# ThomasK33/kube-scheduler-simulator

Hardware: AMD Instinct MI355X
Metric: pod x node filter+score evals/sec (higher is better)
Workload: dtype int64

## Files before the change

### kube-scheduler-simulator_amd/csrc/ksim_batch.hip

```cpp
#include "ksim_device.h"
#include <atomic>

#include "ksim_internal.h"
#include "ksim_wave.h"
#include "ksim_commit.h"
#include "ksim_chain.h"

namespace ksim {



template <int kTopThreads, int N = kTileCand, bool SORTED = true>
__device__ __forceinline__ void top_finish(uint64_t (&a)[N], int32_t nfeas, int32_t j,
                                           uint64_t* __restrict__ topk, int32_t* __restrict__ topk_cnt,
                                           int32_t* __restrict__ topk_complete, uint64_t* __restrict__ xsend,
                                           uint64_t* tclk = nullptr) {
  constexpr int kTopWaves = kTopThreads / 64;
  constexpr int kTopSlots = (kTopWaves * kTopT + 63) / 64;
  __shared__ uint64_t s_list[kTopWaves][kTopT];
  __shared__ int32_t s_cnt[kTopWaves], s_complete[kTopWaves];
  const int lane = threadIdx.x & 63, wv = threadIdx.x >> 6;
  {
    __shared__ uint64_t s_wmax[kTopWaves], s_wthr[kTopWaves];
    __shared__ int32_t s_wf[kTopWaves], s_ncand;
// ... 713 lines not shown
                                          int32_t end) {
  PodRec r{};
  if (q < end) {
    const ksim_pod& y = P.pods[q];
    r.req = PodReq{y.req_cpu, y.req_mem, y.req_eph, y.nz_cpu, y.nz_mem};
    r.cls = rcls[q];
    r.valid = 1;
  }
  return r;
}

template <bool FLUSH, bool DIRECT, bool DEF, bool KEEP, bool NS, bool RT = false>
__device__ __forceinline__ void batch_top_commit_body(const DevCluster& c, const DevPods& P,
                                                      const ksim_profile* __restrict__ prof_p,
                                                      const BatchProg* __restrict__ bp_p, const LazyStep& L,
                                                      uint64_t* __restrict__ topk, int32_t* __restrict__ topk_cnt,
                                                      int32_t* __restrict__ topk_complete,
                                                      int32_t* __restrict__ chosen_out,
                                                      uint64_t* __restrict__ xsend, const ReqTab& rt = ReqTab{}) {
  constexpr int kThreads = 1024;
  static_assert(kThreads >= kBatchPods, "one thread per batch entry");
  static_assert(!RT || (DIRECT && !NS && (FLUSH || (DEF && KEEP))), "the table form is the KEEP / DEF / DIRECT launch");
  static_assert(2 * kReqMaxClasses <= kThreads, "upkeep: one thread per (class, row)");
  __shared__ uint16_t s_cls[RT ? kBatchPods + 1 : 1];
  __shared__ uint16_t s_patch[RT ? kBatchPods + 1 : 1];
  __shared__ UpRow s_up[RT ? 2 : 1];
  __shared__ ResCols s_rq[kBatchPods + 1];
  __shared__ PodReq s_pc[kBatchPods + (NS ? kNsPods : 1)];
  __shared__ __attribute__((aligned(16))) int16_t s_ent[DIRECT ? kLazyDirect : 1];
  __shared__ int32_t s_hkey[DIRECT ? 1 : kLazyHash];
  __shared__ int16_t s_hval[DIRECT ? 1 : kLazyHash];
  __shared__ uint32_t s_bits[DIRECT ? 1 : kLazyBitWords];
  __shared__ int32_t s_istar, s_inode, s_sched, s_unsched;
  const int tid = threadIdx.x;
  const int32_t b = blockIdx.x;
  const int32_t pod0 = NS ? (b / kNsSlices) * kNsPods : b;
#ifdef KSIM_TC_CLOCKS
  const uint64_t t_in = __builtin_amdgcn_s_memrealtime();
  uint64_t t_pro = 0, t_loop = 0, tclk[4] = {0, 0, 0, 0}, tp[3] = {0, 0, 0};
#endif
  const int32_t e1 = *L.e1, e2 = *L.e2;
  uint64_t g1 = 0, m1 = 0, g2 = 0;
  if (tid < kBatchPods) {
    g1 = L.g1[tid];
    m1 = L.m1[tid];
  }
  if (tid == b) g2 = L.g2[b];
  const int32_t cur0 = L.st_in->cursor, end = L.st_in->end;
  const int64_t seq0 = L.st_in->pod_seq;
  ResCols rq{0, 0, 0, 0, 0, 0};
  if constexpr (RT) {
    static_assert(2 * kBatchPods + 1 <= kThreads, "one record per thread");
    if (tid < 2 * kBatchPods + 1) {
      const PodRec r = load_rec(rt.h_in + (tid < kBatchPods ? tid : b + (tid - kBatchPods)));
      if (tid < kBatchPods) {
        rq = ResCols{r.req.cpu, r.req.mem, r.req.eph, r.req.nzc, r.req.nzm, (int32_t)r.valid};
      } else {
        s_pc[tid - kBatchPods] = r.req;
        s_cls[tid - kBatchPods] = r.valid ? r.cls : kNoClass;
      }
    }
  } else {
    for (int x = tid; x < 2 * kBatchPods + (NS ? kNsPods : 1); x += kThreads) {
      const int32_t q = x < kBatchPods ? cur0 + x : cur0 + pod0 + (x - kBatchPods);
      if (q < end) {
        const ksim_pod& y = P.pods[q];
// ... 6 lines not shown
    }
  }
  if constexpr (DIRECT) {
    const uint64_t fill = 0x0001000100010001ull * (uint64_t)kBatchPods;
    for (int x = tid; x < (c.n + 3) >> 2; x += kThreads) reinterpret_cast<uint64_t*>(s_ent)[x] = fill;
  } else {
    const int nwords = (c.n + 31) >> 5;
    for (int x = tid; x < kLazyHash; x += kThreads) s_hkey[x] = -1;
    for (int x = tid; x < nwords; x += kThreads) s_bits[x] = 0;
  }
  const int32_t nchain = e1 > 0 ? e1 : 0;
  if (tid == 0) {
    s_istar = nchain;
    s_inode = -1;
    s_sched = 0;
    s_unsched = 0;
    s_rq[kBatchPods] = ResCols{0, 0, 0, 0, 0, 0};
  }
  PodReq creq{0, 0, 0, 0, 0};
  if constexpr (RT) {
    const int32_t t = tid < 64 ? 0 : tid - 64;
    creq = rt.rreq[t < 2 * rt.n_cls ? (t < rt.n_cls ? t : t - rt.n_cls) : 0];
  }
  lds_barrier();
#ifdef KSIM_TC_CLOCKS
  tp[0] = __builtin_amdgcn_s_memrealtime();
#endif
  block_first_min(&s_istar, tid < nchain && m1 > g1);
  lds_barrier();
#ifdef KSIM_TC_CLOCKS
  tp[1] = __builtin_amdgcn_s_memrealtime();
#endif
  const int32_t istar = s_istar;
  const int32_t committed = istar < nchain ? istar + 1 : nchain;
  if (tid == istar && istar < nchain) s_inode = key_node(m1) - c.base;
  if (tid < committed) s_rq[tid] = rq;
  const int32_t base = cur0 + committed;
  const int32_t pi = base + pod0;
  const bool live = !FLUSH && pi < min(end, base + kBatchPods);
  const int rl = tid - (kThreads - 128);
  const bool rec_writer = RT && rl >= 0 && rl < (int)(sizeof(PodRec) / 8);
  lds_barrier();
#ifdef KSIM_TC_CLOCKS
  tp[2] = __builtin_amdgcn_s_memrealtime();
#endif
  const int32_t inode = s_inode;
  const int32_t gnode = (tid < istar && g1) ? key_node(g1) - c.base : -1;
  uint32_t te[kKeepPerLane];
  uint32_t pe = 0;
  NodeRow prow{};
  double pic = 0, pim = 0;
  const bool twice = RT && !FLUSH && live && gnode >= 0 && gnode == inode;
  if constexpr (RT && !FLUSH) {
    const int32_t cls = live ? (int32_t)s_cls[committed] : 0;
    if (live && gnode >= 0) pe = rt.p_in[(size_t)cls * kBatchPods + tid];
    if (twice) {
      prow = load_res_row_off(c, gnode);
      pic = ld_off(c.inv_cpu, (uint32_t)gnode << 3);
      pim = ld_off(c.inv_mem, (uint32_t)gnode << 3);
    }
    const uint16_t* __restrict__ trow = rt.t_in + (size_t)cls * (size_t)c.n;
#pragma unroll
    for (int q = 0; q < kKeepPerLane; q++) {
      const int32_t node = c.eval_lo + tid + q * kThreads;
      te[q] = trow[node < c.eval_hi ? node : c.eval_lo];
    }
  }
  if (gnode >= 0) {
    ResCols d = rq;
    if (gnode == inode) {
      const ResCols x = s_rq[istar];
      d.cpu += x.cpu;
      d.mem += x.mem;
      d.eph += x.eph;
      d.nzc += x.nzc;
      d.nzm += x.nzm;
      d.pods += 1;
    }
    s_rq[tid] = d;
    if constexpr (RT && !FLUSH) {
// ... 36 lines not shown
    if (mn0 >= 0) mr0 = ResCols{c.req_cpu[mn0], c.req_mem[mn0], c.req_eph[mn0], c.nz_cpu[mn0], c.nz_mem[mn0], c.num_pods[mn0]};
    if (mn1 >= 0) mr1 = ResCols{c.req_cpu[mn1], c.req_mem[mn1], c.req_eph[mn1], c.nz_cpu[mn1], c.nz_mem[mn1], c.num_pods[mn1]};
    if constexpr (RT) {
      const int32_t mn[2] = {mn0, mn1};
#pragma unroll
      for (int w = 0; w < 2; w++) {
        const int32_t n = mn[w] >= 0 ? mn[w] : 0;
        ms[w].alloc_cpu = c.alloc_cpu[n];
        ms[w].alloc_mem = c.alloc_mem[n];
        ms[w].alloc_eph = c.alloc_eph[n];
        ms[w].inv_cpu = c.inv_cpu[n];
        ms[w].inv_mem = c.inv_mem[n];
        ms[w].alloc_pods = c.alloc_pods[n];
        ms[w].node = mn[w];
      }
    }
  }
  lds_barrier();
  auto update_state = [&]() {
    static_assert(sizeof(DevState) % 8 == 0, "DevState by words");
    constexpr int kWords = (int)(sizeof(DevState) / 8);
    uint64_t w[kWords];
#pragma unroll
    for (int q = 0; q < kWords; q++) w[q] = reinterpret_cast<const uint64_t*>(L.st_in)[q];
    DevState ns;
    __builtin_memcpy(&ns, w, sizeof(ns));
    if (e1 > 0) {
      const int32_t nb = min(kBatchPods, end - cur0);
      ns.cursor = base;
      ns.pod_seq = seq0 + committed;
      ns.scheduled += s_sched;
      ns.unschedulable += s_unsched;
      ns.batches += 1;
      ns.cuts += (committed < nb && istar < nchain ? 1 : 0);
      ns.truncations += (committed < nb && istar >= nchain ? 1 : 0);
      ns.evals += (int64_t)committed * (c.eval_hi - c.eval_lo);
    }
    __builtin_memcpy(w, &ns, sizeof(ns));
#pragma unroll
    for (int q = 0; q < kWords; q++) reinterpret_cast<uint64_t*>(L.st_out)[q] = w[q];
    if (L.prog) *L.prog = lazy_progress(ns.cursor, ns.batches);
    if (FLUSH) *L.e_self = -1;
  };
  const bool st_writer = b == 0 && tid == kThreads - 64;
  auto write_records = [&]() {
    if constexpr (RT) {
      static_assert(offsetof(ksim_pod, req_cpu) == 0 && offsetof(ksim_pod, nz_mem) == 32, "ksim_pod starts as PodReq");
      const int32_t q = base + kBatchPods + b;
      uint64_t rec2 = 0;
      if (q < end)
        rec2 = rl < 5 ? reinterpret_cast<const uint64_t*>(&P.pods[q])[rl] : ((uint64_t)rt.rcls[q] | (1ull << 16));
      uint64_t own = 0;
      if (pi < end)
        own = rl < 5 ? reinterpret_cast<const uint64_t*>(&s_pc[committed])[rl]
                     : ((uint64_t)s_cls[committed] | (1ull << 16));
      reinterpret_cast<uint64_t*>(rt.h_out + b)[rl] = own;
      reinterpret_cast<uint64_t*>(rt.h_out + kBatchPods + b)[rl] = rec2;
    }
  };
  auto delta = [&](int32_t node) -> ResCols {
    if constexpr (DIRECT) {
      return s_rq[s_ent[node]];
    } else {
      ResCols d{0, 0, 0, 0, 0, 0};
      const uint32_t bw = s_bits[node >> 5], bit = 1u << (node & 31);
      if (bw & bit) {
        uint32_t h = lazy_hash(node);
        while (s_hkey[h] != node) h = (h + 1) & (kLazyHash - 1);
// ... 204 lines not shown
#ifdef KSIM_TC_CLOCKS
  t_loop = __builtin_amdgcn_s_memrealtime();
#endif
  materialize();
#ifdef KSIM_TC_CLOCKS
  if constexpr (KEEP)
    top_finish<kThreads, kKeepPerLane, false>(ak, nfeas, b, topk, topk_cnt, topk_complete, xsend, tclk);
  else
    top_finish<kThreads>(a, nfeas, b, topk, topk_cnt, topk_complete, xsend, tclk);
  if (tid == 0) {
    const uint64_t t_out = __builtin_amdgcn_s_memrealtime();
    atomicAdd(&g_cp_dbg[0], (unsigned long long)(t_pro - t_in));
    atomicAdd(&g_cp_dbg[1], (unsigned long long)(t_loop - t_pro));
    atomicAdd(&g_cp_dbg[2], (unsigned long long)(tclk[0] - t_loop));
    atomicAdd(&g_cp_dbg[3], (unsigned long long)(t_out - tclk[0]));
    atomicAdd(&g_cp_dbg[4], (unsigned long long)(tp[0] - t_in));
    atomicAdd(&g_cp_dbg[5], 1ull);
    atomicAdd(&g_cp_dbg[6], (unsigned long long)(tp[1] - tp[0]));
    atomicAdd(&g_cp_dbg[7], (unsigned long long)(tp[2] - tp[1]));
  }
#else
  if constexpr (KEEP)
    top_finish<kThreads, kKeepPerLane, false>(ak, nfeas, b, topk, topk_cnt, topk_complete, xsend);
  else
    top_finish<kThreads>(a, nfeas, b, topk, topk_cnt, topk_complete, xsend);
#endif
  upkeep();
  if (rec_writer) write_records();
  if (st_writer) update_state();
  }
}

template <bool FLUSH, bool DIRECT, bool DEF = false, bool KEEP = false, bool NS = false, bool RT = false>
__global__ __launch_bounds__(1024) void k_batch_top_commit(DevCluster c, DevPods P,
                                                           const ksim_profile* __restrict__ prof_p,
                                                           const BatchProg* __restrict__ bp_p, LazyStep L,
                                                           uint64_t* __restrict__ topk, int32_t* __restrict__ topk_cnt,
                                                           int32_t* __restrict__ topk_complete,
                                                           int32_t* __restrict__ chosen_out,
                                                           uint64_t* __restrict__ xsend, ReqTab rt) {
  batch_top_commit_body<FLUSH, DIRECT, DEF, KEEP, NS, RT>(c, P, prof_p, bp_p, L, topk, topk_cnt, topk_complete,
                                                          chosen_out, xsend, rt);
}

__device__ __forceinline__ DevCluster sweep_cols(DevCluster c, const DynCols& d) {
  c.req_cpu = d.req_cpu;
  c.req_mem = d.req_mem;
  c.req_eph = d.req_eph;
  c.nz_cpu = d.nz_cpu;
  c.nz_mem = d.nz_mem;
  c.num_pods = d.num_pods;
  return c;
}

template <bool FLUSH, bool DEF>
__global__ __launch_bounds__(1024) void k_sweep_top_commit(DevCluster c, DevPods P,
                                                           const SweepLane* __restrict__ tab) {
  const SweepLane& r = tab[blockIdx.y];
  const DevCluster cl = sweep_cols(c, r.x_in);
  batch_top_commit_body<FLUSH, true, DEF, !FLUSH, false>(cl, P, r.prof, r.bp, r.step, r.topk, r.topk_cnt,
                                                         r.topk_complete, r.chosen, nullptr);
}

template <bool DEF>
__global__ __launch_bounds__(kBatchPods) void k_sweep_chain_pairs(DevCluster c, DevPods P,
                                                                  const SweepLane* __restrict__ tab) {
  const SweepLane& r = tab[blockIdx.y];
// ... 246 lines not shown
```

### kube-scheduler-simulator_amd/csrc/ksim_device.h

```cpp
#pragma once

#include <hip/hip_runtime.h>
#include <stdint.h>

#include "../../include/ksim_engine.h"

namespace ksim {

constexpr int kMaxNodeScore = 100;

struct DevCluster {
  int32_t n, n_scalar, n_label_cols, n_taints;
  int32_t n_label_values, n_prefer_taints, base, n_total;
  int32_t eval_lo, eval_hi;
  int32_t count_whole;
  uint32_t fit_ignore;
  const int64_t* alloc_cpu;
  const int64_t* alloc_mem;
  const int64_t* alloc_eph;
  const int32_t* alloc_pods;
  const int64_t* alloc_scalar;
  int64_t* req_cpu;
  int64_t* req_mem;
  int64_t* req_eph;
// ... 47 lines not shown
  int64_t* ptab;
  const int4* ptab_ent;
  const int32_t* ptab_cfirst;
  const int32_t* ptab_cidx;
  const int4* ptab_padd;
  int32_t n_pods, n_exprs, n_terms, n_uses, n_adds, n_nn, n_ptab, _pad;
  const int32_t* sclass = nullptr;
  const uint64_t* stab = nullptr;
  int32_t stab_fast = 0, _pad2 = 0;
};

__host__ __device__ __forceinline__ uint64_t stab_word(bool pass, int64_t tt, uint32_t match) {
  return (pass ? (1ull << 63) : 0ull) | ((uint64_t)(tt & 0x7fffffff) << 32) | (uint64_t)match;
}
__host__ __device__ __forceinline__ bool stab_pass(uint64_t w) { return (w >> 63) != 0; }

constexpr int32_t kPtabPlain = 0;
constexpr int32_t kPtabMark = 1;
constexpr int32_t kPtabTotal = 2;

struct DevState {
  int32_t cursor;
  int32_t end;
  int32_t next_start;
  int32_t truncations;
  int64_t pod_seq;
  int64_t evals;
  int64_t scheduled;
  int64_t unschedulable;
  int32_t chosen, status, n_feasible, n_evaluated, n_processed, k_to_find, next_start_after, batches;
  int64_t cuts;
  uint32_t topo_flags;
  int32_t bcap;
};

constexpr uint32_t kTopoAffinityNonEmpty = 1u;
constexpr uint32_t kTopoScoreNonEmpty = 2u;

constexpr int kDomMarkShift = 40;
constexpr int64_t kDomCountMask = (1ll << kDomMarkShift) - 1;

struct BRow;

constexpr int kVarDom = 4;
constexpr int kVarSlots = kVarDom + 1;
struct TbVar {
  int32_t use;
  int32_t adder;
  int32_t nslot;
  int32_t ndom;
  int32_t col;
  int32_t vcol;
  uint32_t zmask;
  int32_t slot_of[kVarSlots];
  uint32_t mask[kVarSlots];
};
struct TbDom {
  int32_t nfeas, nign;
  uint64_t ext[2 * KSIM_MAX_SCORE];
};

constexpr int kExtCut = 2 * KSIM_MAX_SCORE;
constexpr int kExtWords = kExtCut + 1;
struct WinState {
  int32_t cut, kend, nf, evaluated, k, has_soft;
  int32_t nfeas, nign;
// ... 1647 lines not shown
```

### kube-scheduler-simulator_amd/csrc/ksim_engine.cpp

```cpp
#include <dlfcn.h>
#include <hip/hip_runtime.h>
#include <rccl/rccl.h>

#include <algorithm>
#include <array>
#include <chrono>
#include <cstdio>
#include <cstdlib>
#include <cstring>
#include <map>
#include <string>
#include <tuple>
#include <unordered_map>
#include <type_traits>
#include <vector>

#include "ksim_internal.h"

using namespace ksim;

namespace {

constexpr int kGraphCycles = 128;

// ... 208 lines not shown
  hipGraphExec_t graph_lazy_adapt = nullptr;
  hipGraphExec_t graph_lazy4 = nullptr, graph_lazy4_adapt = nullptr, graph_lazy4_rt = nullptr;
  unsigned long long* prog = nullptr;
  unsigned long long* prog_d = nullptr;
  bool counters_pending = false;
  int64_t feed_syncs = 0, feed_past_end = 0, feed_fallbacks = 0, feed_topups = 0, feed_odd_ends = 0;
  std::vector<uint16_t> rq_cls;
  uint16_t* d_rcls = nullptr;
  PodReq* d_rreq = nullptr;
  int32_t rq_ncls = 0;
  std::vector<DevBuf> rtab_bufs;
  size_t rtab_bytes = 0;
  hipGraphExec_t graph_lazy_rt = nullptr;
  int64_t rtab_runs = 0;
  int32_t rt_graph_ncls = 0;
  std::vector<DevBuf> ash_bufs;
  uint64_t *ash_send = nullptr, *ash_recv = nullptr, *ash_gmask = nullptr;
  int32_t ash_world = 0, ash_w = 0;
  struct SweepLaneBufs {
    DynCols x[2];
    uint64_t *g, *m;
    int32_t* e;
    uint64_t* topk;
    int32_t *topk_cnt, *topk_complete, *pinv;
    int64_t* pnorm;
  };
  void* sweep_slab = nullptr;
  int32_t sweep_n = -1, sweep_lanes = 0;
  std::vector<SweepLaneBufs> sweep_lane;
  DevState* sweep_st = nullptr;
  SweepLane* sweep_tab = nullptr;
  DevArena sweep_profs, sweep_rows;
  std::map<std::pair<int32_t, bool>, hipGraphExec_t> sweep_graphs;
  int64_t graph_captures = 0;
  int64_t graph_gen = 0;
  std::vector<std::pair<const ksim_handle*, int64_t>> sg_sig;
  std::map<std::tuple<bool, int64_t, int64_t>, hipGraphExec_t> sg_graphs;
  bool sg_off = false;
  int64_t match_ns = 0;
};

namespace {

int set_err(ksim_handle* h, int code, const std::string& msg) {
  if (h) h->err = msg;
  return code;
}

int hip_fail(ksim_handle* h, hipError_t e, const char* what) {
  int code = (e == hipErrorOutOfMemory) ? KSIM_E_OOM : KSIM_E_DEVICE;
  return set_err(h, code, std::string(what) + ": " + hipGetErrorString(e));
}

#define HIPCHK(h, expr)                                    \
  do {                                                     \
    hipError_t _e = (expr);                                \
    if (_e != hipSuccess) return hip_fail((h), _e, #expr); \
  } while (0)

static hipError_t hcopy(ksim_handle* h, void* dst, const void* src, size_t bytes, hipMemcpyKind kind) {
  const hipError_t e = hipMemcpyAsync(dst, src, bytes, kind, h->stream);
  return e != hipSuccess ? e : hipStreamSynchronize(h->stream);
}

static hipError_t hzero(ksim_handle* h, void* dst, size_t bytes) {
  const hipError_t e = hipMemsetAsync(dst, 0, bytes, h->stream);
// ... 450 lines not shown
    }
    h->graph_captures++;
  }
  int32_t cursor = a;
  while (cursor < b) {
    int32_t nbat = 0;
    for (int32_t i = cursor; i < b; nbat++) i += std::min(std::min(kTbPods, b - i), std::max(h->tlen[i], 1));
    int32_t done = 0;
    for (; done + kGraphBatches <= nbat; done += kGraphBatches) HIPCHK(h, hipGraphLaunch(h->graph_tbatch, h->stream));
    for (; done < nbat; done++) launch_tbatch(la, h->stream);
    HIPCHK(h, hipGetLastError());
    DevState st;
    if ((rc = read_state(h, st))) return rc;
    if (st.cursor <= cursor) return set_err(h, KSIM_E_DEVICE, "topology batch path made no progress");
    cursor = st.cursor;
  }
  return KSIM_OK;
}

bool lazy_enabled() {
  constexpr bool off = ab(kAbLazy);
  return !off;
}

bool lazy_ok(const ksim_handle* h, int32_t a, int32_t b, bool fast, bool stab = false) {
  if (!lazy_enabled() || !fast || stab) return false;
  if (adapt_mode(h) ? (is_sharded(h) && !h->replicated) : (is_sharded(h) || h->replicated)) return false;
  if (h->dc.base != 0 || h->dc.n > kLazyMaxNodes || h->dc.n <= 0) return false;
  for (int32_t i = a; i < b; i++)
    if (!h->noadd[i]) return false;
  return true;
}

int alloc_lazy(ksim_handle* h) {
  if (h->lazy_n == h->dc.n) return KSIM_OK;
  HIPCHK(h, hipStreamSynchronize(h->stream));
  drop_lazy_graphs(h);
  free_bufs(h->lazy_bufs);
  h->lazy_n = -1;
  if (!h->prog) {
    hipError_t e = hipHostMalloc((void**)&h->prog, 2 * sizeof(unsigned long long), hipHostMallocCoherent | hipHostMallocMapped);
    if (e != hipSuccess) {
      h->prog = nullptr;
      return hip_fail(h, e, "hipHostMalloc (progress word)");
    }
    h->prog[0] = h->prog[1] = 0;
    if ((e = hipHostGetDevicePointer((void**)&h->prog_d, h->prog, 0)) != hipSuccess)
      return hip_fail(h, e, "hipHostGetDevicePointer");
  }
  const size_t n = (size_t)h->dc.n;
  int rc;
  void* p = nullptr;
  int64_t** cols[5] = {&h->lazy_x1.req_cpu, &h->lazy_x1.req_mem, &h->lazy_x1.req_eph, &h->lazy_x1.nz_cpu,
                       &h->lazy_x1.nz_mem};
  for (auto* c : cols) {
    if ((rc = upload(h, h->lazy_bufs, nullptr, 8 * n, &p))) return rc;
    *c = (int64_t*)p;
  }
  if ((rc = upload(h, h->lazy_bufs, nullptr, 4 * n, &p))) return rc;
  h->lazy_x1.num_pods = (int32_t*)p;
  if ((rc = upload(h, h->lazy_bufs, nullptr, sizeof(DevState), &p))) return rc;
  h->lazy_st1 = (DevState*)p;
  if ((rc = upload(h, h->lazy_bufs, nullptr, 8 * (size_t)kLazySlots * kBatchPods, &p))) return rc;
  h->lazy_g = (uint64_t*)p;
  if ((rc = upload(h, h->lazy_bufs, nullptr, 8 * (size_t)kLazySlots * kBatchPods, &p))) return rc;
  h->lazy_m = (uint64_t*)p;
  if ((rc = upload(h, h->lazy_bufs, nullptr, 4 * (size_t)kLazySlots, &p))) return rc;
// ... 44 lines not shown
}
int ensure_rtab(ksim_handle* h) {
  const size_t need = rtab_halves_bytes(h) + rtab_patch_bytes(h) + sizeof(PodRec) * 2 * 2 * kBatchPods;
  if (h->rtab_bytes >= need && !h->rtab_bufs.empty()) return KSIM_OK;
  HIPCHK(h, hipStreamSynchronize(h->stream));
  drop_lazy_pair(h->graph_lazy_rt, h->graph_lazy4_rt);
  free_bufs(h->rtab_bufs);
  h->rtab_bytes = 0;
  void* p = nullptr;
  int rc;
  if ((rc = upload(h, h->rtab_bufs, nullptr, need, &p))) return rc;
  h->rtab_bytes = need;
  return KSIM_OK;
}

LazyBatch lazy_batch(const ksim_handle* h, const LaunchArgs& la, int64_t i, bool rt = false) {
  const int p = (int)(i & 1), q = (int)(i & 3), q1 = (int)((i + 3) & 3), q2 = (int)((i + 2) & 3);
  const DynCols x[2] = {dyn_cols(h->dc), h->lazy_x1};
  DevState* st[2] = {h->st, h->lazy_st1};
  LazyBatch z;
  z.a = la;
  z.a.c = with_cols(la.c, x[p ^ 1]);
  z.cw = with_cols(la.c, x[p]);
  z.step.w = x[p];
  z.step.st_in = st[p ^ 1];
  z.step.st_out = st[p];
  z.step.g1 = h->lazy_g + (size_t)q1 * kBatchPods;
  z.step.m1 = h->lazy_m + (size_t)q1 * kBatchPods;
  z.step.e1 = h->lazy_e + q1;
  z.step.g2 = h->lazy_g + (size_t)q2 * kBatchPods;
  z.step.e2 = h->lazy_e + q2;
  z.step.e_self = h->lazy_e + q;
  z.step.prog = h->prog_d;
  z.st = st[p];
  z.gkey = h->lazy_g + (size_t)q * kBatchPods;
  z.pmax = h->lazy_m + (size_t)q * kBatchPods;
  z.cend = h->lazy_e + q;
  z.b1 = h->lazy_ab + (size_t)q1 * kBatchPods;
  z.w1 = h->lazy_aw + (size_t)q1 * 2 * kBatchPods;
  z.abroken = h->lazy_ab + (size_t)q * kBatchPods;
  z.awin = h->lazy_aw + (size_t)q * 2 * kBatchPods;
  if (rt) {
    uint16_t* const t = (uint16_t*)h->rtab_bufs[0].p;
    const size_t half = (size_t)h->rq_ncls * (size_t)h->dc.n;
    z.rt.t_in = t + (size_t)(p ^ 1) * half;
    z.rt.t_out = t + (size_t)p * half;
    z.rt.rreq = h->d_rreq;
    z.rt.rcls = h->d_rcls;
    z.rt.n_cls = h->rq_ncls;
    uint16_t* const pe = (uint16_t*)((char*)h->rtab_bufs[0].p + rtab_halves_bytes(h));
    const size_t slot = (size_t)h->rq_ncls * kBatchPods;
    z.rt.p_in = pe + (size_t)q1 * slot;
    z.rt.p_out = pe + (size_t)q * slot;
    PodRec* const rec = (PodRec*)((char*)pe + rtab_patch_bytes(h));
    z.rt.h_in = rec + (size_t)(p ^ 1) * 2 * kBatchPods;
    z.rt.h_out = rec + (size_t)p * 2 * kBatchPods;
  }
  return z;
}

int lazy_begin(ksim_handle* h) {
  int rc;
  if ((rc = alloc_lazy(h))) return rc;
  const size_t n = (size_t)h->dc.n;
  const DynCols x0 = dyn_cols(h->dc), x1 = h->lazy_x1;
  HIPCHK(h, hipMemcpyAsync(x1.req_cpu, x0.req_cpu, 8 * n, hipMemcpyDeviceToDevice, h->stream));
// ... 190 lines not shown
        __builtin_ia32_pause();
      }
    }
    if (news) {
      cursor = (int32_t)(last >> 32);
      done = (int32_t)((uint32_t)last - (uint32_t)word[1]);
    } else {
      if (!forced) {
        const hipError_t q = hipStreamQuery(h->stream);
        if (q != hipSuccess && q != hipErrorNotReady) return hip_fail(h, q, "hipStreamQuery");
      }
      lazy_flush(h, lazy_batch(h, la, i, rt), h->stream);
      HIPCHK(h, hipGetLastError());
      DevState st;
      if ((rc = read_state_at(h, (i & 1) ? h->lazy_st1 : h->st, st))) return rc;
      h->feed_syncs++;
      h->feed_fallbacks++;
      i++;
      flushed = true;
      last = word[0];
      if (st.cursor <= cursor) return set_err(h, KSIM_E_DEVICE, "deferred-commit batch path made no progress");
      cursor = st.cursor;
      done = launched;
    }
    if (cursor < b && (rc = act(true))) return rc;
  }
  if (!flushed) return set_err(h, KSIM_E_DEVICE, "deferred-commit run ended without its flush");
  h->feed_past_end += launched - done;
  h->feed_odd_ends += (i - 1) & 1;
  return lazy_end_run(h, i - 1);
}

int alloc_sweep(ksim_handle* h, int32_t lanes) {
  if (!h->sweep_tab) {
    void* t = nullptr;
    hipError_t e = hipMalloc(&t, sizeof(SweepLane) * kLazySlots * kSweepMaxLanes);
    if (e != hipSuccess) return hip_fail(h, e, "hipMalloc");
    h->sweep_tab = (SweepLane*)t;
  }
  if (h->sweep_n == h->dc.n && lanes <= h->sweep_lanes) return KSIM_OK;
  HIPCHK(h, hipStreamSynchronize(h->stream));
  if (h->sweep_slab) (void)hipFree(h->sweep_slab);
  h->sweep_slab = nullptr;
  h->sweep_n = -1;
  h->sweep_lanes = 0;
  h->sweep_lane.clear();
  const size_t n = (size_t)h->dc.n;
  size_t off = 0;
  auto take = [&](size_t bytes) {
    const size_t at = off;
    off += (bytes + 255) & ~(size_t)255;
    return at;
  };
  struct Off {
    size_t col[2][6], g, m, e, topk, cnt, cmp, pnorm, pinv;
  };
  std::vector<Off> offs((size_t)lanes);
  const size_t st_off = take(sizeof(DevState) * 2 * (size_t)lanes);
  for (auto& o : offs) {
    for (int p = 0; p < 2; p++)
      for (int k = 0; k < 6; k++) o.col[p][k] = take(k < 5 ? 8 * n : 4 * n);
    o.g = take(8 * (size_t)kLazySlots * kBatchPods);
    o.m = take(8 * (size_t)kLazySlots * kBatchPods);
    o.e = take(4 * (size_t)kLazySlots);
    o.topk = take(8 * (size_t)kBatchPods * kTopT);
    o.cnt = take(4 * (size_t)kBatchPods);
// ... 32 lines not shown
}

int sweep_reserve(ksim_handle* h, DevArena& a, size_t bytes) {
  if (a.cap >= bytes && a.p) return KSIM_OK;
  HIPCHK(h, hipStreamSynchronize(h->stream));
  if (a.p) (void)hipFree(a.p);
  a.p = nullptr;
  a.cap = 0;
  const hipError_t e = hipMalloc(&a.p, bytes ? bytes : 16);
  if (e != hipSuccess) {
    a.p = nullptr;
    return hip_fail(h, e, "hipMalloc");
  }
  a.cap = bytes ? bytes : 16;
  return KSIM_OK;
}

SweepLane sweep_record(const ksim_handle* h, int32_t l, int q, int32_t* row, const ksim_profile* prof,
                       const BatchProg* bp) {
  const ksim_handle::SweepLaneBufs& b = h->sweep_lane[(size_t)l];
  const int p = q & 1, q1 = (q + 3) & 3, q2 = (q + 2) & 3;
  DevState* st[2] = {h->sweep_st + 2 * (size_t)l, h->sweep_st + 2 * (size_t)l + 1};
  SweepLane r{};
  r.x_in = b.x[p ^ 1];
  r.step.w = b.x[p];
  r.step.st_in = st[p ^ 1];
  r.step.st_out = st[p];
  r.step.g1 = b.g + (size_t)q1 * kBatchPods;
  r.step.m1 = b.m + (size_t)q1 * kBatchPods;
  r.step.e1 = b.e + q1;
  r.step.g2 = b.g + (size_t)q2 * kBatchPods;
  r.step.e2 = b.e + q2;
  r.step.e_self = b.e + q;
  r.gkey = b.g + (size_t)q * kBatchPods;
  r.pmax = b.m + (size_t)q * kBatchPods;
  r.topk = b.topk;
  r.topk_cnt = b.topk_cnt;
  r.topk_complete = b.topk_complete;
  r.pnorm = b.pnorm;
  r.pinv = b.pinv;
  r.chosen = row;
  r.prof = prof;
  r.bp = bp;
  return r;
}

int run_sweep(ksim_handle* h, int32_t a, int32_t b, int32_t n_profs, int32_t lanes, bool def,
              const ksim_profile* d_profs, const BatchProg* d_bps, int32_t* chosen, ksim_batch_stats* stats) {
  int rc;
  if ((rc = alloc_sweep(h, lanes))) return rc;
  const int32_t np = h->dp.n_pods, count = b - a;
  if ((rc = sweep_reserve(h, h->sweep_rows, 4 * (size_t)lanes * (size_t)std::max(np, 1)))) return rc;
  int32_t* rows = (int32_t*)h->sweep_rows.p;
  LaunchArgs la = make_args(h, h->dp, nullptr);
  const DevCluster c = la.c;
  const DevPods P = h->dp;
  SweepLane* const tab = h->sweep_tab;
  std::vector<SweepLane> htab((size_t)kLazySlots * kSweepMaxLanes);
  std::vector<int32_t> vec((size_t)lanes, -1), cur((size_t)lanes, 0);
  std::vector<DevState> hst(2 * (size_t)lanes);
  int32_t next_v = 0, live = 0;
  DevState st0[2] = {}, idle[2] = {};
  st0[0].cursor = st0[1].cursor = a;
  st0[0].end = st0[1].end = b;
  auto arm = [&](int32_t l, int32_t v) -> int {
    const ksim_handle::SweepLaneBufs& B = h->sweep_lane[(size_t)l];
// ... 679 lines not shown
  }
  return KSIM_OK;
}

int shard_schedule(const std::vector<ksim_handle*>& hs, int32_t first, int32_t count) {
  if (profile_nb(hs[0]->prof))
    return set_err(hs[0], KSIM_E_UNSUPPORTED, "NetworkBandwidth profiles run on unsharded handles");
  if (hs[0]->replicated) {
    const bool adapt = adapt_mode(hs[0]);
    return for_each_run(hs[0], first, count, [&](int32_t a, int32_t b, bool batch, bool topo) {
      if (batch && !adapt) return topo ? shard_run_tbatch(hs, a, b) : shard_run(hs, a, b);
      for (auto* h : hs) {
        int rc = run_range(h, a, b, batch, topo);
        if (rc) return rc;
      }
      return (int)KSIM_OK;
    }, true);
  }
  const bool adapt = adapt_mode(hs[0]);
  const bool adapt_batch = adapt && adapt_shard_layout(hs);
  return for_each_run(hs[0], first, count, [&](int32_t a, int32_t b, bool batch, bool) {
    if (!batch) return shard_run_perpod(hs, a, b);
    return adapt ? shard_run_adapt(hs, a, b) : shard_run(hs, a, b);
  }, adapt_batch);
}



int reset_counters(ksim_handle* h, hipStream_t stream) {
  HIPCHK(h, hipMemsetAsync(&h->st->truncations, 0, 4, stream));
  HIPCHK(h, hipMemsetAsync(&h->st->evals, 0, 3 * sizeof(int64_t), stream));
  HIPCHK(h, hipMemsetAsync(&h->st->batches, 0, 4, stream));
  HIPCHK(h, hipMemsetAsync(&h->st->cuts, 0, 8, stream));
  return KSIM_OK;
}

}

extern "C" {

int ksim_abi_version(void) { return KSIM_ABI_VERSION; }

size_t ksim_abi_sizeof(int which) {
  switch (which) {
    case 0: return sizeof(ksim_node_table);
    case 1: return sizeof(ksim_vocab);
    case 2: return sizeof(ksim_label_expr);
    case 3: return sizeof(ksim_term);
    case 4: return sizeof(ksim_pod);
    case 5: return sizeof(ksim_pod_set);
    case 6: return sizeof(ksim_profile);
    case 7: return sizeof(ksim_eval_out);
    case 8: return sizeof(ksim_batch_stats);
    case 9: return sizeof(ksim_topo_use);
    case 10: return sizeof(ksim_class_add);
    case 11: return sizeof(ksim_match_problem);
    case 12: return sizeof(ksim_k8s_kv);
    case 13: return sizeof(ksim_k8s_taint);
    case 14: return sizeof(ksim_k8s_toleration);
    case 15: return sizeof(ksim_k8s_requirement);
    case 16: return sizeof(ksim_k8s_selector_term);
    case 17: return sizeof(ksim_k8s_preferred_term);
    case 18: return sizeof(ksim_k8s_label_selector);
    case 19: return sizeof(ksim_k8s_pod_term);
    case 20: return sizeof(ksim_k8s_spread);
    case 21: return sizeof(ksim_k8s_port);
// ... 2537 lines not shown
      DevState st;
      if ((r = read_state(h, st))) return r;
      const int32_t did = batch ? std::min<int32_t>(iters, st.batches) : std::min(iters, st.cursor - cursor);
      for (int32_t i = 0; i < did; i++)
        for (int k = 0; k < per; k++) {
          if (!((launched >> k) & 1u)) continue;
          float ms = 0;
          const size_t b = (size_t)i * (per + 1);
          HIPCHK(h, hipEventElapsedTime(&ms, evs[b + k], evs[b + k + 1]));
          sum[base + k] += ms;
          n[base + k] += 1;
        }
      for (auto& e : evs) (void)hipEventDestroy(e);
      if (st.cursor <= cursor) return set_err(h, KSIM_E_DEVICE, "no progress while timing");
      cursor = st.cursor;
    }
    return KSIM_OK;
  });
  if (rc) return rc;
  for (int k = 0; k < kKinds; k++) {
    avg_ms[k] = n[k] ? sum[k] / n[k] : 0.0;
    if (launches) launches[k] = n[k];
  }
  return kKinds;
}

}

extern "C" int ksim_get_diag(ksim_handle* h, int64_t* out, int32_t n) {
  if (!h || !out || n < 0) return KSIM_E_INVALID;
  DevState st;
  int rc = read_state(h, st);
  if (rc) return rc;
  int64_t v[3 + 16 + 2 + 4 + 3 + 5] = {st.batches, st.truncations, st.cuts};
  if (h->has_cluster) HIPCHK(h, hcopy(h, v + 3, h->sc.dbg, 8 * 16, hipMemcpyDeviceToHost));
  if (unsigned long long* cp = cp_clock_buffer())
    HIPCHK(h, hcopy(h, v + 3, cp, 8 * 8, hipMemcpyDeviceToHost));
  if (unsigned long long* ad = adapt_dbg_buffer())
    HIPCHK(h, hcopy(h, v + 3, ad, 8 * 8, hipMemcpyDeviceToHost));
  v[19] = h->graph_captures;
  v[20] = h->match_ns;
  for (int k = 0; k < 4; k++) v[21 + k] = h->fw_counts[k];
  v[25] = (int64_t)batch_variant_reach();
  if (h->has_cluster && h->sc.tb_vpods) HIPCHK(h, hcopy(h, v + 26, h->sc.tb_vpods, 8, hipMemcpyDeviceToHost));
  v[27] = h->rtab_runs;
  v[28] = h->feed_syncs;
  v[29] = h->feed_past_end;
  v[30] = h->feed_fallbacks;
  v[31] = h->feed_topups;
  v[32] = h->feed_odd_ends;
  const int32_t m = n < 33 ? n : 33;
  for (int32_t i = 0; i < m; i++) out[i] = v[i];
  return m;
}

extern "C" int32_t ksim_feed_more_batches(int32_t left, int32_t pending) {
  return lazy_more_batches(left, pending, kBatchPods);
}

extern "C" int ksim_batch_geometry(int32_t* out, int32_t n) {
  if (!out || n < 0) return KSIM_E_INVALID;
  const int32_t v[4] = {kBatchPods, kTopT, kTopThreads, kTileCand};
  const int32_t m = n < 4 ? n : 4;
  for (int32_t i = 0; i < m; i++) out[i] = v[i];
  return m;
}


extern "C" int ksim_set_bound_pods(ksim_handle* h, const ksim_bound_pods* b) {
  int rc = ensure_ready(h);
  if (rc) return rc;
  if (!b || b->n < 0 || (b->n > 0 && (!b->node || !b->priority || !b->start_time || !b->req)))
    return set_err(h, KSIM_E_INVALID, "bad bound-pod table");
  const int32_t N = h->dc.n, n = b->n;
  for (int32_t i = 0; i < n; i++)
    if (b->node[i] < 0 || b->node[i] >= N) return set_err(h, KSIM_E_INVALID, "bound pod on a node out of range");
  std::vector<int32_t> ix((size_t)n);
  for (int32_t i = 0; i < n; i++) ix[i] = i;
  std::sort(ix.begin(), ix.end(), [&](int32_t x, int32_t y) {
    if (b->node[x] != b->node[y]) return b->node[x] < b->node[y];
    if (b->priority[x] != b->priority[y]) return b->priority[x] > b->priority[y];
    if (b->start_time[x] != b->start_time[y]) return b->start_time[x] < b->start_time[y];
    return x < y;
  });
// ... 407 lines not shown
```

### kube-scheduler-simulator_amd/csrc/ksim_internal.h

```cpp
#pragma once

#include "ksim_device.h"

namespace ksim {

constexpr unsigned kAbStab = 1;
constexpr unsigned kAbLazy = 2;
constexpr unsigned kAbAdaptNorm = 4;
constexpr unsigned kAbTbatch = 8;
constexpr unsigned kAbShardGraph = 16;
constexpr unsigned kAbPtab = 32;
constexpr unsigned kAbTbVar = 64;
constexpr unsigned kAbReqTab = 128;
#ifdef KSIM_AB_FORMS
constexpr unsigned kAbMask = KSIM_AB_FORMS;
#else
constexpr unsigned kAbMask = 0;
#endif
constexpr bool ab(unsigned form) { return (kAbMask & form) != 0; }


#ifndef KSIM_BATCH_PODS
#define KSIM_BATCH_PODS 256
#endif
// ... 66 lines not shown
constexpr int kLazyMaxNodes = 1 << 17;
constexpr int kLazyHashBits = 10;
struct DynCols {
  int64_t *req_cpu, *req_mem, *req_eph, *nz_cpu, *nz_mem;
  int32_t* num_pods;
};
constexpr int kReqMaxClasses = 256;
struct alignas(16) PodRec {
  PodReq req;
  uint16_t cls, valid;
  uint32_t _pad;
};
static_assert(sizeof(PodRec) == 48, "pod record: three 16-byte words");
constexpr uint16_t kNoClass = 0xffff;
struct ReqTab {
  const uint16_t* t_in = nullptr;
  uint16_t* t_out = nullptr;
  const PodReq* rreq = nullptr;
  const uint16_t* rcls = nullptr;
  const uint16_t* p_in = nullptr;
  uint16_t* p_out = nullptr;
  const PodRec* h_in = nullptr;
  PodRec* h_out = nullptr;
  int32_t n_cls = 0, _pad = 0;
};
struct LazyStep {
  DynCols w;
  const DevState* st_in;
  DevState* st_out;
  const uint64_t* g1; const uint64_t* m1; const int32_t* e1;
  const uint64_t* g2; const int32_t* e2;
  int32_t* e_self;
  unsigned long long* prog = nullptr;
};
__host__ __device__ inline unsigned long long lazy_progress(int32_t cursor, int32_t batches) {
  return ((unsigned long long)(uint32_t)cursor << 32) | (uint32_t)batches;
}
constexpr int32_t lazy_more_batches(int32_t left, int32_t pending, int32_t batch_pods) {
  return left <= 0 ? 0 : ((left - 1) / batch_pods + 1 > pending ? (left - 1) / batch_pods + 1 - pending : 0);
}
struct LazyBatch {
  LaunchArgs a;
  DevCluster cw;
  LazyStep step;
  ReqTab rt;
  DevState* st;
  uint64_t* gkey;
  uint64_t* pmax;
  int32_t* cend;
  const int32_t* b1;
  const int32_t* w1;
  int32_t* abroken;
  int32_t* awin;
};
constexpr int kSweepMaxLanes = 64;
struct SweepLane {
  DynCols x_in;
  LazyStep step;
  uint64_t* gkey;
  uint64_t* pmax;
  uint64_t* topk;
  int32_t* topk_cnt;
  int32_t* topk_complete;
  int64_t* pnorm;
  int32_t* pinv;
  int32_t* chosen;
// ... 143 lines not shown
```

### kube-scheduler-simulator_amd/csrc/ksim_kernels.hip

```cpp
#include "ksim_device.h"
#include "ksim_internal.h"
#include "ksim_wave.h"
#include "ksim_cycle.h"

namespace ksim {

__device__ __forceinline__ uint64_t wave_max_u64(uint64_t v) {
#pragma unroll
  for (int m = 32; m >= 1; m >>= 1) {
    uint64_t o = shfl_xor_u64(v, m);
    v = o > v ? o : v;
  }
  return v;
}

__device__ __forceinline__ int64_t wave_max_i64(int64_t v) {
#pragma unroll
  for (int m = 32; m >= 1; m >>= 1) {
    int64_t o = (int64_t)shfl_xor_u64((uint64_t)v, m);
    v = o > v ? o : v;
  }
  return v;
}

// ... 991 lines not shown

__global__ __launch_bounds__(256) void k_lazy_move(LazyMove m) {
  const int32_t stride = (int32_t)(gridDim.x * blockDim.x);
  const int32_t t0 = (int32_t)(blockIdx.x * blockDim.x + threadIdx.x);
  for (int32_t i = t0; i < m.n; i += stride) {
    const int64_t a = m.src.req_cpu[i], b = m.src.req_mem[i], c = m.src.req_eph[i], d = m.src.nz_cpu[i],
                  e = m.src.nz_mem[i];
    const int32_t f = m.src.num_pods[i];
    m.dst.req_cpu[i] = a;
    m.dst.req_mem[i] = b;
    m.dst.req_eph[i] = c;
    m.dst.nz_cpu[i] = d;
    m.dst.nz_mem[i] = e;
    m.dst.num_pods[i] = f;
  }
  if (m.begin) {
    static_assert(sizeof(WinState) % 4 == 0, "WinState by words");
    for (int32_t i = t0; i < (int32_t)(sizeof(WinState) / 4); i += stride) reinterpret_cast<uint32_t*>(m.win)[i] = 0u;
    if (blockIdx.x == 0 && threadIdx.x < kLazySlots) m.ring_e[threadIdx.x] = -1;
  }
  if (blockIdx.x == 0 && threadIdx.x == 0) {
    DevState s = *m.st_src;
    if (m.begin) {
      s.cursor = m.first;
      s.end = m.end;
      s.bcap = 0;
      if (m.zero_counters) {
        s.truncations = 0;
        s.evals = 0;
        s.scheduled = 0;
        s.unschedulable = 0;
        s.batches = 0;
        s.cuts = 0;
      }
      *m.st_dst2 = s;
      if (m.batches0) *m.batches0 = (unsigned long long)(uint32_t)s.batches;
    }
    *m.st_dst = s;
  }
}

void launch_lazy_move(const LazyMove& m, hipStream_t stream) {
  const int blocks = std::min(256, std::max(1, (m.n + 255) / 256));
  k_lazy_move<<<blocks, 256, 0, stream>>>(m);
}

__global__ void k_assume(DevCluster c, DevPods P, int32_t pod, int32_t node, int sign) {
  if (threadIdx.x == 0 && blockIdx.x == 0) assume_pod(c, P, P.pods[pod], node, sign);
}


__global__ __launch_bounds__(256) void k_dom_pack(DevCluster c, DevPods P, const DevState* __restrict__ st,
                                                  DevScratch s) {
  const int32_t pi = st->cursor;
  if (pi >= st->end) return;
  const ksim_pod& p = P.pods[pi];
  int64_t off = 0;
  for (int i = 0; i < p.use_count; i++) {
    const ksim_topo_use u = P.uses[p.use_first + i];
    if (!use_needs_dom(u)) continue;
    const int32_t V = c.col_nvals[u.col];
    const int64_t* d = s.dom + (size_t)i * c.vmax;
    for (int32_t v = threadIdx.x; v < V; v += blockDim.x) s.xdom[off + v] = d[v];
    off += V;
  }
}
// ... 497 lines not shown
```

### kube-scheduler-simulator_amd/ksim/engine.py

```python
from __future__ import annotations

import ctypes
import os
from typing import Optional

import numpy as np

from . import abi

_HERE = os.path.dirname(os.path.abspath(__file__))
_VARIANT = os.environ.get("KSIM_LIB_VARIANT", "")
LIB_PATH = os.path.join(_HERE, f"libksim_engine_{_VARIANT}.so" if _VARIANT else "libksim_engine.so")
_LIB = None

EXPORTS = [
    "ksim_abi_version", "ksim_abi_sizeof", "ksim_create", "ksim_destroy", "ksim_last_error",
    "ksim_set_profile", "ksim_set_cluster", "ksim_get_node_state", "ksim_get_class_count", "ksim_get_nb_alloc", "ksim_get_next_start",
    "ksim_set_next_start", "ksim_set_pod_seq", "ksim_eval_pod", "ksim_assume", "ksim_forget",
    "ksim_load_pods", "ksim_schedule_loaded", "ksim_schedule_batch", "ksim_reset_cluster", "ksim_sweep_loaded",
    "ksim_time_kernels", "ksim_kernel_name", "ksim_time_eval", "ksim_get_diag", "ksim_batch_geometry",
    "ksim_set_shard", "ksim_comm_unique_id", "ksim_comm_init", "ksim_group_schedule_loaded",
    "ksim_emit_cycle_json", "ksim_eval_pod_filter", "ksim_eval_pod_finish",
    "ksim_set_bound_pods", "ksim_set_bound_pod_adds", "ksim_set_bound_pod_pdbs", "ksim_preempt", "ksim_upsert_nodes", "ksim_remove_node",
    "ksim_match_terms", "ksim_set_eval_range", "ksim_fw_prefilter", "ksim_fw_score", "ksim_fw_normalize",
# ... 440 lines not shown
        V = len(profiles)
        arr = (abi.Profile * max(V, 1))(*profiles)
        chosen = np.zeros((V, max(count, 0)), np.int32)
        stats = (abi.BatchStats * max(V, 1))()
        self._chk(self.L.ksim_sweep_loaded(self.h, first, count, arr, V, max_lanes,
                                           chosen.ctypes.data_as(ctypes.c_void_p), stats))
        return chosen, [stats[v] for v in range(V)]

    def node_state(self) -> dict:
        n = self.n_nodes
        out = {k: np.zeros(n, np.int64) for k in ("req_cpu", "req_mem", "req_eph", "nz_cpu", "nz_mem")}
        out["num_pods"] = np.zeros(n, np.int32)
        a = [out[k].ctypes.data_as(ctypes.c_void_p) for k in
             ("req_cpu", "req_mem", "req_eph", "nz_cpu", "nz_mem", "num_pods")]
        self._chk(self.L.ksim_get_node_state(self.h, *a))
        return out

    @property
    def next_start(self) -> int:
        v = ctypes.c_int32()
        self._chk(self.L.ksim_get_next_start(self.h, ctypes.byref(v)))
        return v.value

    def set_next_start(self, s: int):
        self._chk(self.L.ksim_set_next_start(self.h, s))

    def set_pod_seq(self, s: int):
        self._chk(self.L.ksim_set_pod_seq(self.h, s))

    def reset_cluster(self):
        self._chk(self.L.ksim_reset_cluster(self.h))

    def diag(self) -> dict:
        out = np.zeros(33, np.int64)
        n = self.L.ksim_get_diag(self.h, out.ctypes.data_as(ctypes.c_void_p), 33)
        if n < 0:
            self._chk(n)
        d = {"batches": int(out[0]), "truncations": int(out[1]), "cuts": int(out[2]),
             "graph_captures": int(out[19]), "dbg": [int(x) for x in out[3:19]], "match_ns": int(out[20]),
             "fw_score_host": int(out[21]), "fw_score_device": int(out[22]), "fw_normalize_cached": int(out[23]),
             "fw_normalize_device": int(out[24]), "variants": int(out[25]), "tb_variant_pods": int(out[26]),
             "reqtab_runs": int(out[27]),
             "feed_syncs": int(out[28]), "feed_past_end": int(out[29]), "feed_fallbacks": int(out[30]),
             "feed_topups": int(out[31]), "feed_odd_ends": int(out[32])}
        if out[6]:
            d["chain_us"] = {"setup": out[3] / out[6] / 100.0, "rounds": out[4] / out[6] / 100.0,
                             "epilogue": out[5] / out[6] / 100.0, "rounds_per_batch": out[7] / out[6]}
        return d

    def time_eval(self, first: int, reps: int = 200):
        ms = ctypes.c_double()
        k = ctypes.c_int32()
        self._chk(self.L.ksim_time_eval(self.h, first, reps, ctypes.byref(ms), ctypes.byref(k)))
        return self.L.ksim_kernel_name(k.value).decode(), ms.value

    def time_kernels(self, first: int, count: int) -> dict:
        out = np.zeros(32, np.float64)
        cnt = np.zeros(32, np.int64)
        n = self.L.ksim_time_kernels(self.h, first, count, out.ctypes.data_as(ctypes.c_void_p),
                                    cnt.ctypes.data_as(ctypes.c_void_p), 32)
        if n < 0:
            self._chk(n)
        return {self.L.ksim_kernel_name(k).decode(): (float(out[k]), int(cnt[k]))
                for k in range(n) if cnt[k] > 0}


class _EmitInput(ctypes.Structure):
    _fields_ = [("n_nodes", ctypes.c_int32), ("n_filter", ctypes.c_int32), ("n_score", ctypes.c_int32),
                ("n_messages", ctypes.c_int32),
                ("node_names", ctypes.c_void_p), ("filter_names", ctypes.c_void_p),
                ("score_names", ctypes.c_void_p), ("score_weight", ctypes.c_void_p),
                ("has_normalize", ctypes.c_void_p), ("fail_plugin", ctypes.c_void_p),
                ("msg_id", ctypes.c_void_p), ("messages", ctypes.c_void_p), ("scored", ctypes.c_void_p),
                ("raw", ctypes.c_void_p), ("norm", ctypes.c_void_p)]


def _cstrs(names):
# ... 37 lines not shown
```

Measured before the change: 47.62 billion.

## Stretch batch commit past the first conflict when later pods stay valid

After the first pod whose best key is invalidated (istar), the commit kernel re-checks later pods in the chain. Each one re-scores the conflicting node (with the accumulated requests added) and its own chosen node, and the batch keeps committing until the first pod whose choice changes. The aim is to commit more pods per batch and so run fewer batches and relaunches. It adds extra node-row loads, scoring and barriers per batch, plus new stretch counters, and an env flag (KSIM_ONE_CUT) restores the old single-cut behaviour. Launch bounds also gain a minimum-blocks hint, which may constrain register allocation.

After: 51.32 billion, median of 6. 7.8% higher.

```diff
diff --git a/kube-scheduler-simulator_amd/csrc/ksim_batch.hip b/kube-scheduler-simulator_amd/csrc/ksim_batch.hip
--- a/kube-scheduler-simulator_amd/csrc/ksim_batch.hip
+++ b/kube-scheduler-simulator_amd/csrc/ksim_batch.hip
@@ -769,6 +769,8 @@
   __shared__ int16_t s_hval[DIRECT ? 1 : kLazyHash];
   __shared__ uint32_t s_bits[DIRECT ? 1 : kLazyBitWords];
   __shared__ int32_t s_istar, s_inode, s_sched, s_unsched;
+  __shared__ int32_t s_fnode, s_i2;
+  __shared__ ResCols s_dd;
   const int tid = threadIdx.x;
   const int32_t b = blockIdx.x;
   const int32_t pod0 = NS ? (b / kNsSlices) * kNsPods : b;
@@ -841,9 +843,82 @@
   tp[1] = __builtin_amdgcn_s_memrealtime();
 #endif
   const int32_t istar = s_istar;
-  const int32_t committed = istar < nchain ? istar + 1 : nchain;
+  int32_t committed = istar < nchain ? istar + 1 : nchain;
   if (tid == istar && istar < nchain) s_inode = key_node(m1) - c.base;
   if (tid < committed) s_rq[tid] = rq;
+  const bool stretch = !L.one_cut && istar + 1 < nchain;
+  if (stretch) {
+    if (tid == istar) {
+      s_fnode = g1 ? key_node(g1) - c.base : -1;
+      s_i2 = nchain;
+    }
+    lds_barrier();
+    const int32_t nn = s_inode, fn = s_fnode;
+    const bool mine = tid > istar && tid < nchain;
+    NodeRow rn{}, rf{};
+    double icn = 0, imn = 0, icf = 0, imf = 0;
+    if (!FLUSH && mine) {
+      const int32_t ff = fn >= 0 ? fn : nn;
+      rn = load_res_row_off(c, nn);
+      icn = ld_off(c.inv_cpu, (uint32_t)nn << 3);
+      imn = ld_off(c.inv_mem, (uint32_t)nn << 3);
+      rf = load_res_row_off(c, ff);
+      icf = ld_off(c.inv_cpu, (uint32_t)ff << 3);
+      imf = ld_off(c.inv_mem, (uint32_t)ff << 3);
+    }
+    if (tid < istar && g1 && key_node(g1) - c.base == nn) {
+      const ResCols x = s_rq[istar];
+      s_dd = ResCols{rq.cpu + x.cpu, rq.mem + x.mem, rq.eph + x.eph, rq.nzc + x.nzc, rq.nzm + x.nzm, rq.pods + x.pods};
+    }
+    lds_barrier();
+    bool ends = false;
+    if (mine) {
+      const ResCols d = s_dd;
+      rn.req_cpu += d.cpu;
+      rn.req_mem += d.mem;
+      rn.req_eph += d.eph;
+      rn.nz_cpu += d.nzc;
+      rn.nz_mem += d.nzm;
+      rn.num_pods += d.pods;
+      ksim_pod pq;
+      pq.req_cpu = rq.cpu;
+      pq.req_mem = rq.mem;
+      pq.req_eph = rq.eph;
+      pq.nz_cpu = rq.nzc;
+      pq.nz_mem = rq.nzm;
+#pragma unroll
+      for (int k = 0; k < KSIM_MAX_SCALAR; k++) pq.scalar_req[k] = 0;
+      const FastProg bq = fast_prog(*bp_p);
+      const uint64_t hs = prof_p->tiebreak_seed ^ ((uint64_t)(seq0 + tid) << 20);
+      if constexpr (FLUSH) {
+        uint64_t k2 = m1;
+#pragma unroll 1
+        for (int w = 0; w < 2; w++) {
+          const int32_t node = w ? fn : nn;
+          if (node < 0) continue;
+          NodeRow r = load_res_row_off(c, node);
+          const double ic = ld_off(c.inv_cpu, (uint32_t)node << 3), im = ld_off(c.inv_mem, (uint32_t)node << 3);
+          if (w == 0) {
+            r.req_cpu += d.cpu;
+            r.req_mem += d.mem;
+            r.req_eph += d.eph;
+            r.nz_cpu += d.nzc;
+            r.nz_mem += d.nzm;
+            r.num_pods += d.pods;
+          }
+          k2 = umax64(k2, dyn_key_fast_t<DEF>(bq, pq, r, ic, im, hs, c.base + node));
+        }
+        ends = k2 > g1;
+      } else {
+        const uint64_t dk = dyn_key_fast_t<DEF>(bq, pq, rn, icn, imn, hs, c.base + nn);
+        const uint64_t fk = fn >= 0 ? dyn_key_fast_t<DEF>(bq, pq, rf, icf, imf, hs, c.base + fn) : 0;
+        ends = umax64(umax64(m1, dk), fk) > g1;
+      }
+    }
+    block_first_min(&s_i2, ends);
+    lds_barrier();
+    committed = s_i2;
+  }
   const int32_t base = cur0 + committed;
   const int32_t pi = base + pod0;
   const bool live = !FLUSH && pi < min(end, base + kBatchPods);
@@ -854,7 +929,7 @@
   tp[2] = __builtin_amdgcn_s_memrealtime();
 #endif
   const int32_t inode = s_inode;
-  const int32_t gnode = (tid < istar && g1) ? key_node(g1) - c.base : -1;
+  const int32_t gnode = (tid < committed && tid != istar && g1) ? key_node(g1) - c.base : -1;
   uint32_t te[kKeepPerLane];
   uint32_t pe = 0;
   NodeRow prow{};
@@ -957,8 +1032,13 @@
       ns.scheduled += s_sched;
       ns.unschedulable += s_unsched;
       ns.batches += 1;
-      ns.cuts += (committed < nb && istar < nchain ? 1 : 0);
-      ns.truncations += (committed < nb && istar >= nchain ? 1 : 0);
+      const bool pair_end = istar < nchain && (!stretch || committed < nchain);
+      ns.cuts += (committed < nb && pair_end ? 1 : 0);
+      ns.truncations += (committed < nb && !pair_end ? 1 : 0);
+      if (stretch && committed > istar + 1) {
+        ns.stretches += 1;
+        ns.stretch_pods += committed - (istar + 1);
+      }
       ns.evals += (int64_t)committed * (c.eval_hi - c.eval_lo);
     }
     __builtin_memcpy(w, &ns, sizeof(ns));
@@ -1229,7 +1309,7 @@
 }
 
 template <bool FLUSH, bool DIRECT, bool DEF = false, bool KEEP = false, bool NS = false, bool RT = false>
-__global__ __launch_bounds__(1024) void k_batch_top_commit(DevCluster c, DevPods P,
+__global__ __launch_bounds__(1024, (FLUSH && !DIRECT) ? 8 : 4) void k_batch_top_commit(DevCluster c, DevPods P,
                                                            const ksim_profile* __restrict__ prof_p,
                                                            const BatchProg* __restrict__ bp_p, LazyStep L,
                                                            uint64_t* __restrict__ topk, int32_t* __restrict__ topk_cnt,
diff --git a/kube-scheduler-simulator_amd/csrc/ksim_device.h b/kube-scheduler-simulator_amd/csrc/ksim_device.h
--- a/kube-scheduler-simulator_amd/csrc/ksim_device.h
+++ b/kube-scheduler-simulator_amd/csrc/ksim_device.h
@@ -103,6 +103,7 @@
   int64_t cuts;
   uint32_t topo_flags;
   int32_t bcap;
+  int32_t stretches, stretch_pods;
 };
 
 constexpr uint32_t kTopoAffinityNonEmpty = 1u;
diff --git a/kube-scheduler-simulator_amd/csrc/ksim_engine.cpp b/kube-scheduler-simulator_amd/csrc/ksim_engine.cpp
--- a/kube-scheduler-simulator_amd/csrc/ksim_engine.cpp
+++ b/kube-scheduler-simulator_amd/csrc/ksim_engine.cpp
@@ -264,6 +264,7 @@
   SweepLane* sweep_tab = nullptr;
   DevArena sweep_profs, sweep_rows;
   std::map<std::pair<int32_t, bool>, hipGraphExec_t> sweep_graphs;
+  bool one_cut = false;
   int64_t graph_captures = 0;
   int64_t graph_gen = 0;
   std::vector<std::pair<const ksim_handle*, int64_t>> sg_sig;
@@ -780,7 +781,23 @@
   return true;
 }
 
+int sync_one_cut(ksim_handle* h) {
+  const char* v = std::getenv("KSIM_ONE_CUT");
+  const bool want = v && v[0] == '1';
+  if (want == h->one_cut) return KSIM_OK;
+  HIPCHK(h, hipStreamSynchronize(h->stream));
+  drop_lazy_graphs(h);
+  for (auto& kv : h->sweep_graphs)
+    if (kv.second) (void)hipGraphExecDestroy(kv.second);
+  h->sweep_graphs.clear();
+  for (auto& kv : h->sg_graphs) (void)hipGraphExecDestroy(kv.second);
+  h->sg_graphs.clear();
+  h->one_cut = want;
+  return KSIM_OK;
+}
+
 int alloc_lazy(ksim_handle* h) {
+  if (int rc = sync_one_cut(h)) return rc;
   if (h->lazy_n == h->dc.n) return KSIM_OK;
   HIPCHK(h, hipStreamSynchronize(h->stream));
   drop_lazy_graphs(h);
@@ -891,6 +908,7 @@
   z.step.e2 = h->lazy_e + q2;
   z.step.e_self = h->lazy_e + q;
   z.step.prog = h->prog_d;
+  z.step.one_cut = h->one_cut ? 1 : 0;
   z.st = st[p];
   z.gkey = h->lazy_g + (size_t)q * kBatchPods;
   z.pmax = h->lazy_m + (size_t)q * kBatchPods;
@@ -1147,6 +1165,7 @@
 }
 
 int alloc_sweep(ksim_handle* h, int32_t lanes) {
+  if (int rc = sync_one_cut(h)) return rc;
   if (!h->sweep_tab) {
     void* t = nullptr;
     hipError_t e = hipMalloc(&t, sizeof(SweepLane) * kLazySlots * kSweepMaxLanes);
@@ -1245,6 +1264,7 @@
   r.step.g2 = b.g + (size_t)q2 * kBatchPods;
   r.step.e2 = b.e + q2;
   r.step.e_self = b.e + q;
+  r.step.one_cut = h->one_cut ? 1 : 0;
   r.gkey = b.g + (size_t)q * kBatchPods;
   r.pmax = b.m + (size_t)q * kBatchPods;
   r.topk = b.topk;
@@ -1990,6 +2010,8 @@
   HIPCHK(h, hipMemsetAsync(&h->st->evals, 0, 3 * sizeof(int64_t), stream));
   HIPCHK(h, hipMemsetAsync(&h->st->batches, 0, 4, stream));
   HIPCHK(h, hipMemsetAsync(&h->st->cuts, 0, 8, stream));
+  static_assert(offsetof(DevState, stretch_pods) == offsetof(DevState, stretches) + 4, "the stretch counters are adjacent");
+  HIPCHK(h, hipMemsetAsync(&h->st->stretches, 0, 8, stream));
   return KSIM_OK;
 }
 
@@ -4593,7 +4615,7 @@
   DevState st;
   int rc = read_state(h, st);
   if (rc) return rc;
-  int64_t v[3 + 16 + 2 + 4 + 3 + 5] = {st.batches, st.truncations, st.cuts};
+  int64_t v[3 + 16 + 2 + 4 + 3 + 5 + 2] = {st.batches, st.truncations, st.cuts};
   if (h->has_cluster) HIPCHK(h, hcopy(h, v + 3, h->sc.dbg, 8 * 16, hipMemcpyDeviceToHost));
   if (unsigned long long* cp = cp_clock_buffer())
     HIPCHK(h, hcopy(h, v + 3, cp, 8 * 8, hipMemcpyDeviceToHost));
@@ -4610,7 +4632,9 @@
   v[30] = h->feed_fallbacks;
   v[31] = h->feed_topups;
   v[32] = h->feed_odd_ends;
-  const int32_t m = n < 33 ? n : 33;
+  v[33] = st.stretches;
+  v[34] = st.stretch_pods;
+  const int32_t m = n < 35 ? n : 35;
   for (int32_t i = 0; i < m; i++) out[i] = v[i];
   return m;
 }
diff --git a/kube-scheduler-simulator_amd/csrc/ksim_internal.h b/kube-scheduler-simulator_amd/csrc/ksim_internal.h
--- a/kube-scheduler-simulator_amd/csrc/ksim_internal.h
+++ b/kube-scheduler-simulator_amd/csrc/ksim_internal.h
@@ -122,6 +122,7 @@
   const uint64_t* g2; const int32_t* e2;
   int32_t* e_self;
   unsigned long long* prog = nullptr;
+  int32_t one_cut = 0, _pad = 0;
 };
 __host__ __device__ inline unsigned long long lazy_progress(int32_t cursor, int32_t batches) {
   return ((unsigned long long)(uint32_t)cursor << 32) | (uint32_t)batches;
diff --git a/kube-scheduler-simulator_amd/csrc/ksim_kernels.hip b/kube-scheduler-simulator_amd/csrc/ksim_kernels.hip
--- a/kube-scheduler-simulator_amd/csrc/ksim_kernels.hip
+++ b/kube-scheduler-simulator_amd/csrc/ksim_kernels.hip
@@ -1047,6 +1047,8 @@
         s.unschedulable = 0;
         s.batches = 0;
         s.cuts = 0;
+        s.stretches = 0;
+        s.stretch_pods = 0;
       }
       *m.st_dst2 = s;
       if (m.batches0) *m.batches0 = (unsigned long long)(uint32_t)s.batches;
diff --git a/kube-scheduler-simulator_amd/ksim/engine.py b/kube-scheduler-simulator_amd/ksim/engine.py
--- a/kube-scheduler-simulator_amd/ksim/engine.py
+++ b/kube-scheduler-simulator_amd/ksim/engine.py
@@ -496,8 +496,8 @@
         self._chk(self.L.ksim_reset_cluster(self.h))
 
     def diag(self) -> dict:
-        out = np.zeros(33, np.int64)
-        n = self.L.ksim_get_diag(self.h, out.ctypes.data_as(ctypes.c_void_p), 33)
+        out = np.zeros(35, np.int64)
+        n = self.L.ksim_get_diag(self.h, out.ctypes.data_as(ctypes.c_void_p), 35)
         if n < 0:
             self._chk(n)
         d = {"batches": int(out[0]), "truncations": int(out[1]), "cuts": int(out[2]),
@@ -506,7 +506,8 @@
              "fw_normalize_device": int(out[24]), "variants": int(out[25]), "tb_variant_pods": int(out[26]),
              "reqtab_runs": int(out[27]),
              "feed_syncs": int(out[28]), "feed_past_end": int(out[29]), "feed_fallbacks": int(out[30]),
-             "feed_topups": int(out[31]), "feed_odd_ends": int(out[32])}
+             "feed_topups": int(out[31]), "feed_odd_ends": int(out[32]),
+             "stretches": int(out[33]), "stretch_pods": int(out[34])}
         if out[6]:
             d["chain_us"] = {"setup": out[3] / out[6] / 100.0, "rounds": out[4] / out[6] / 100.0,
                              "epilogue": out[5] / out[6] / 100.0, "rounds_per_batch": out[7] / out[6]}
```
